# insitro/FastVim

Measured on AMD Instinct MI355X. Metric: images/sec FastVim-T 224px bs=128/GPU fwd+bwd (+all-reduce +AdamW +EMA), whole job, higher is better.
Workload: dtype bf16; 1 GPU; FastVim-T 224x224 bs=128/GPU bf16 training step, synthetic ImageNet tensors (BASELINE configs[1]); global_batch=128, parallelism=dp1, hip_graph=True, optimizer_in_step=True, final_loss_hex=0x1.779ca20000000p+0

## Files before the change

fastvim_amd/_lib.py:

```python
import ctypes
import os
import threading

import torch

_PKG = os.path.dirname(os.path.abspath(__file__))
LIB_PATH = os.path.join(_PKG, "libfastvim_hip.so")

FV_F32, FV_BF16, FV_F16 = 0, 1, 2
_DTYPES = {torch.float32: FV_F32, torch.bfloat16: FV_BF16, torch.float16: FV_F16}

_lib = None

C_ABI_SYMBOLS = (
    "fv_last_error", "fv_version",
    "fv_selective_scan_fwd", "fv_selective_scan_bwd_workspace", "fv_selective_scan_bwd",
    "fv_causal_conv1d_fwd", "fv_causal_conv1d_bwd", "fv_scan_expand_skip_fwd",
    "fv_mixer_conv_pool_fwd", "fv_mixer_scan_fwd", "fv_mixer_xproj_scan_fwd_ok", "fv_mixer_xproj_scan_fwd", "fv_mixer_combine_fwd",
    "fv_mixer_bwd_blocks", "fv_mixer_combine_bwd", "fv_mixer_scan_bwd_chunks", "fv_mixer_scan_bwd_chunks_b",
    "fv_mixer_scan_bwd_ckpt_floats", "fv_mixer_scan_bwd_partials", "fv_mixer_scan_bwd", "fv_mixer_scan_bwd_dir", "fv_mixer_scan_bwd_ckpt", "fv_mixer_scan_bwd_segments", "fv_mixer_scan_bwd_seg_floats", "fv_mixer_scan_bwd_seg_partials", "fv_mixer_scan_bwd_seg_chunks", "fv_mixer_scan_bwd_seg", "fv_mixer_scan_fwd_ckpt", "fv_mixer_scan_ckpt_floats", "fv_mixer_scan_fwd_segments", "fv_mixer_scan_fwd_seg_floats", "fv_mixer_scan_fwd_seg", "fv_rows_segment_sum", "fv_rows_gather", "fv_mixer_conv_pool_bwd", "fv_mixer_conv_pool_bwd2_ok", "fv_mixer_conv_pool_bwd2", "fv_mixer_scan_bwd_xproj_ok", "fv_mixer_scan_bwd_xproj", "fv_chunk_rows_bf16", "fv_reduce_partials", "fv_reduce_partials_multi",
    "fv_add_norm_blocks", "fv_add_norm_fwd", "fv_add_norm_bwd", "fv_gemm_bf16", "fv_gemm_bf16_tn_grouped", "fv_gemm_bf16_tn_grouped_ld", "fv_mixer_xproj_fwd", "fv_mixer_xproj_bwd_slices", "fv_mixer_xproj_bwd", "fv_mixer_xproj_bwd2", "fv_mixer_xproj_bwd3_ok", "fv_mixer_xproj_bwd3", "fv_adamw_flat", "fv_soft_target_ce",
    "fv_patch_unfold", "fv_gemm_bf16_rowbias", "fv_mean_pool_fwd", "fv_mean_pool_bwd", "fv_droppath_table", "fv_scale_cast",
    "fv_column_sum", "fv_gemm_bf16_addnorm", "fv_gemm_bf16_dgrad_addnorm_blocks", "fv_gemm_bf16_dgrad_addnorm_bwd", "fv_gemm_bf16_dgrad_addnorm_bwd2", "fv_gemm_bf16_addnorm2", "fv_mixer_combine_out_proj_addnorm_ok", "fv_mixer_combine_out_proj_addnorm", "fv_gemm_f32",
    "fv_mixer_conv_pool_bwd_dgrad_ok", "fv_mixer_conv_pool_bwd_dgrad_blocks", "fv_mixer_conv_pool_bwd_dgrad", "fv_transpose_bf16_batched", "fv_gemm_bf16_tn_grouped_wide8",
    "fv_grad_sumsq_blocks", "fv_grad_sumsq_partials", "fv_adamw_flat_groups",
    "fv_pack_weight_frags_batched", "fv_mixer_conv_pool_bwd_dgrad_pk", "fv_mixer_combine_out_proj_addnorm_pk",
    "fv_mix_batch", "fv_patch_unfold_mix", "fv_mixup_target", "fv_label_ce",
    "fv_patch_unfold_chan", "fv_chan_embed_table", "fv_chan_embed_scatter",
    "fv_mixer_plan",
    "fv_bn1d_stats", "fv_bn1d_apply", "fv_bn1d_bwd", "fv_sgd_flat", "fv_lars_partials_per_segment", "fv_lars_sumsq_partials", "fv_lars_flat",
    "fv_tap_ln_blocks", "fv_tap_ln_fwd", "fv_tap_ln_bwd", "fv_ln2d_blocks", "fv_ln2d_fwd", "fv_ln2d_bwd",
)


_tls = threading.local()


class _DeviceGuarded:

    def __init__(self, cdll):
        self._cdll = cdll
        self._wrapped = {}

    def __getattr__(self, name):
        w = self._wrapped.get(name)
        if w is None:
            fn = getattr(self._cdll, name)

            def call(*args, _fn=fn):
                dev = getattr(_tls, "dev", None)
                if dev is None or dev == torch.cuda.current_device():
                    return _fn(*args)
                with torch.cuda.device(dev):
                    return _fn(*args)

            w = self._wrapped[name] = call
        return w


def lib():
    global _lib
    if _lib is None:
        if not os.path.exists(LIB_PATH):
            raise RuntimeError(
# ... 44 lines not shown
```

fastvim_amd/csrc/scan_cl.hip:

```cpp
#include <stdlib.h>

#include "common.h"
#include "lane_reduce.h"
#include "scan_step.h"
#include <type_traits>

namespace {

constexpr int N = 16;
constexpr int CPB = 64;

struct ScanClParams {
  const void* xc;
  const void* xdbl;
  const float* Wdt[2];
  const float* dtb[2];
  const float* Alog[2];
  float* yc;
  const float* dyc;
  size_t dyc_dir;
  float* dxc;
  float* dxdbl;
  float* ckpt;
  float* pP;
// ... 1327 lines not shown
  }
}

__global__ __launch_bounds__(256) void scan_seg_combine_kernel(ScanClParams p) {
  const size_t i = (size_t)blockIdx.x * blockDim.x + threadIdx.x;
  const size_t per = (size_t)p.d_in * N, total = (size_t)2 * p.B * per;
  if (i >= total) return;
  const int n = (int)(i % N), d = (int)((i / N) % p.d_in);
  const size_t db = i / per;
  const int dir = (int)(db / p.B);
  const float A = -__expf(p.Alog[dir][(size_t)d * N + n]);
  float* hin = const_cast<float*>(p.hin);
  float H = 0.f;
  for (int k = 0; k < p.seg; ++k) {
    const int s = p.adj ? p.seg - 1 - k : k;
    const size_t sidx = (db * p.seg + s) * p.d_in + d;
    hin[sidx * N + n] = H;
    H = fmaf(__expf(A * p.sumdt[sidx]), H, p.hend[sidx * N + n]);
  }
}

typedef __bf16 sc_bf16x8 __attribute__((ext_vector_type(8)));

template <int RQ, int LCT>
struct ShortFwdLds {
  static constexpr int RQP = (RQ + 3) / 4 * 4, WP = 4 * RQP + 2 * N;
  static constexpr int xc_stride(int d_in) { return d_in * 2 + 16; }
  static constexpr int o_xc = 0;
  static constexpr int o_dbl(int d_in) { return o_xc + 16 * xc_stride(d_in); }
  static constexpr int o_ch(int d_in) { return o_dbl(d_in) + LCT * WP * 4; }
  static constexpr int o_y(int d_in) { return o_ch(d_in) + LCT * SH_CH * 8; }
  static constexpr int o_xp(int d_in) { return o_y(d_in) + LCT * SH_CH * 4; }
  static constexpr int bytes(int d_in, int NT) { return o_xp(d_in) + SH_NWV * NT * 256 * 4; }
};

template <int RQ, int LCT, bool EXACT>
__global__ __launch_bounds__(SH_THREADS) void xproj_scan_fwd_short_kernel(ScanClParams p, const bf16_t* __restrict__ Wx2,
                                                                         bf16_t* __restrict__ xdbl_out, int NT) {
  extern __shared__ __attribute__((aligned(16))) char smc[];
  typedef ShortFwdLds<RQ, LCT> LD;
  constexpr int RQP = LD::RQP, WP = LD::WP;
  const int d_in = p.d_in, W = p.R + 2 * N;
  const int Lc = EXACT ? LCT : p.Lc;
  const int XS = LD::xc_stride(d_in);
  char* s_xc = smc + LD::o_xc;
  float* s_dbl = (float*)(smc + LD::o_dbl(d_in));
  float* s_ch = (float*)(smc + LD::o_ch(d_in));
  float* s_y = (float*)(smc + LD::o_y(d_in));
  float* s_xp = (float*)(smc + LD::o_xp(d_in));
  const int tid = threadIdx.x, lane = tid & 63, wv = tid >> 6;
  const int dir = blockIdx.y, b = blockIdx.x;
  const size_t bd = ((size_t)dir * p.B + b) * Lc;
  struct ChunkPar { float w[RQP]; float bias; float al[4]; };
  auto load_par = [&](int ch0, ChunkPar& c) {
    const int dm = ch0 + wv * 16 + (lane & 15), tg_ = lane >> 4;
    const bool actm = dm < d_in;
    const int ddm = actm ? dm : 0;
    c.bias = p.dtb[dir][ddm];
#pragma unroll
    for (int kg = 0; kg < RQP; ++kg) {
      const int r = 4 * kg + tg_;
      c.w[kg] = (actm && r < p.R) ? p.Wdt[dir][(size_t)ddm * p.R + r] : 0.f;
    }
    const int d = ch0 + wv * 16 + (lane >> 2), dd = d < d_in ? d : 0;
    const float4 a4 = *reinterpret_cast<const float4*>(p.Alog[dir] + (size_t)dd * N + (lane & 3) * 4);
    c.al[0] = a4.x; c.al[1] = a4.y; c.al[2] = a4.z; c.al[3] = a4.w;
  };
  ChunkPar par0, par1;
  load_par(0, par0);
  if (SH_CH < d_in) load_par(SH_CH, par1);
  sc_bf16x8 bw0[7];
  {
    const int r = lane & 15, kc = lane >> 4;
    const bf16_t* Wd = Wx2 + (size_t)dir * W * d_in;
    const int k0 = min(wv, d_in / 32 - 1) * 32 + kc * 8;
#pragma unroll
    for (int nt = 0; nt < 7; ++nt)
      if (nt < NT) bw0[nt] = *reinterpret_cast<const sc_bf16x8*>(Wd + (size_t)min(nt * 16 + r, W - 1) * d_in + k0);
  }
  {
    const bf16_t* xc = (const bf16_t*)p.xc + bd * d_in;
    const int vpr = d_in / 8;
    for (int e = tid; e < 16 * vpr; e += SH_THREADS) {
      const int srow = e / vpr, v = e - srow * vpr;
      uint4 val = make_uint4(0u, 0u, 0u, 0u);
      if (srow < Lc) {
        const int l = dir ? Lc - 1 - srow : srow;
        val = *reinterpret_cast<const uint4*>(xc + (size_t)l * d_in + v * 8);
      }
      *reinterpret_cast<uint4*>(s_xc + srow * XS + v * 16) = val;
    }
    for (int e = tid; e < LCT * WP; e += SH_THREADS) s_dbl[e] = 0.f;
  }
  __syncthreads();
  {
    f32x4_t acc[7];
#pragma unroll
    for (int nt = 0; nt < 7; ++nt) acc[nt] = (f32x4_t){0.f, 0.f, 0.f, 0.f};
    const int r = lane & 15, kc = lane >> 4;
    const bf16_t* Wd = Wx2 + (size_t)dir * W * d_in;
    for (int ks = wv; ks < d_in / 32; ks += SH_NWV) {
      const int k0 = ks * 32 + kc * 8;
      const sc_bf16x8 a = *reinterpret_cast<const sc_bf16x8*>(s_xc + r * XS + k0 * 2);
#pragma unroll
      for (int nt = 0; nt < 7; ++nt) {
        if (nt < NT) {
          const int n = min(nt * 16 + r, W - 1);
          const sc_bf16x8 bw = ks == wv ? bw0[nt] : *reinterpret_cast<const sc_bf16x8*>(Wd + (size_t)n * d_in + k0);
          acc[nt] = __builtin_amdgcn_mfma_f32_16x16x32_bf16(bw, a, acc[nt], 0, 0, 0);
        }
      }
    }
#pragma unroll
    for (int nt = 0; nt < 7; ++nt)
      if (nt < NT) *reinterpret_cast<f32x4_t*>(s_xp + ((size_t)(wv * NT + nt) * 64 + lane) * 4) = acc[nt];
  }
  __syncthreads();
  {
    bf16_t* xo = xdbl_out + bd * W;
    for (int e = tid; e < Lc * W; e += SH_THREADS) {
      const int t = e / W, n = e - t * W;
      const int nt = n >> 4, ln = t + 16 * ((n & 15) >> 2), j = n & 3;
      float v = 0.f;
#pragma unroll
      for (int w = 0; w < SH_NWV; ++w) v += s_xp[((size_t)(w * NT + nt) * 64 + ln) * 4 + j];
      const bf16_t vb = __float2bfloat16(v);
      const int l = dir ? Lc - 1 - t : t;
      xo[(size_t)l * W + n] = vb;
      const int pos = n < p.R ? (n & 3) * RQP + (n >> 2) : 4 * RQP + (n - p.R);
      s_dbl[t * WP + pos] = __bfloat162float(vb);
    }
  }
  __syncthreads();
  const int q = lane & 3, cm = lane & 15, tg = lane >> 4;
  const float* my_bc = s_dbl + 4 * RQP + q * 4;
  auto chunk = [&](int ch0, const ChunkPar& par) {
    {
      const int dm = ch0 + wv * 16 + cm;
      const bool actm = dm < d_in;
      const int ddm = actm ? dm : 0;
      const float bias_m = par.bias;
      f32x4_t D = {0.f, 0.f, 0.f, 0.f};
      const int ta = min(cm, LCT - 1);
#pragma unroll
      for (int kg = 0; kg < RQP; ++kg) {
        const float a = s_dbl[ta * WP + tg * RQP + kg];
        D = __builtin_amdgcn_mfma_f32_16x16x4f32(a, par.w[kg], D, 0, 0, 0);
// ... 29 lines not shown
        asm volatile("" ::: "memory");
        if (EXACT || s < Lc) {
          const float4 Bv = *reinterpret_cast<const float4*>(my_bc + s * WP);
          const float4 Cv = *reinterpret_cast<const float4*>(my_bc + s * WP + N);
          const float2 cv = *reinterpret_cast<const float2*>(my_ch + s * (SH_CH * 2));
          const sf2 Bn[2] = {{Bv.x, Bv.y}, {Bv.z, Bv.w}}, Cn[2] = {{Cv.x, Cv.y}, {Cv.z, Cv.w}};
          sf2 acc2 = {0.f, 0.f};
#pragma unroll
          for (int h = 0; h < 2; ++h) {
            st[h] = sfma2(sexp2_2(A2[h] * cv.x), st[h], Bn[h] * cv.y);
            acc2 = sfma2(Cn[h], st[h], acc2);
          }
          const float acc = quad_sum(acc2.x + acc2.y);
          s_y[s * SH_CH + chl] = acc;
        }
      }
    }
    __builtin_amdgcn_fence(__ATOMIC_RELEASE, "wavefront");
    __builtin_amdgcn_wave_barrier();
    __builtin_amdgcn_fence(__ATOMIC_ACQUIRE, "wavefront");
    {
      const int dm = ch0 + wv * 16 + cm;
#pragma unroll
      for (int r = 0; r < 4; ++r) {
        const int s = 4 * tg + r;
        if (dm < d_in && s < Lc) {
          const int l = dir ? Lc - 1 - s : s;
          p.yc[(bd + l) * d_in + dm] = s_y[s * SH_CH + wv * 16 + cm];
        }
      }
    }
    __builtin_amdgcn_wave_barrier();
  };
  chunk(0, par0);
  if (SH_CH < d_in) chunk(SH_CH, par1);
  for (int ch0 = 2 * SH_CH; ch0 < d_in; ch0 += SH_CH) {
    ChunkPar pc;
    load_par(ch0, pc);
    chunk(ch0, pc);
  }
}

int rq_of(int R) { return (R + 3) / 4; }

}

extern "C" int fv_mixer_scan_fwd(const void* xc, const void* x_dbl, const float* dt_w, const float* dt_bias,
                                 const float* A_log, const float* dt_w_b, const float* dt_bias_b,
                                 const float* A_log_b, float* yc, int batch, int Lc, int d_inner, int dt_rank,
                                 int d_state, int dtype, fv_stream_t stream) {
  return fv_mixer_scan_fwd_ckpt(xc, x_dbl, dt_w, dt_bias, A_log, dt_w_b, dt_bias_b, A_log_b, yc, nullptr, batch, Lc, d_inner,
                                dt_rank, d_state, dtype, stream);
}

extern "C" int fv_mixer_scan_fwd_segments(int batch, int Lc, int d_inner, int dt_rank) {
  static const int force = fv_tune("FASTVIM_SCAN_FWD_SEG", 0);
  const int nchunk = (Lc + 15) / 16;
  if (Lc <= 16 || dt_rank > 48) return 1;
  if (force > 0) {
    const int f = force < nchunk ? force : nchunk, cps = (nchunk + f - 1) / f;
    return (nchunk + cps - 1) / cps;
  }
  const long wgs = (long)fv_cdiv(d_inner, CPB) * batch * 2;
  if (wgs >= 512 || nchunk < 16) return 1;
  long s = (1024 + wgs - 1) / wgs;
  if (s > nchunk / 8) s = nchunk / 8;
  if (s < 1) s = 1;
  const long cps = (nchunk + s - 1) / s;
  return (int)((nchunk + cps - 1) / cps);
}
extern "C" size_t fv_mixer_scan_fwd_seg_floats(int batch, int Lc, int d_inner, int d_state, int dt_rank) {
  const int S = fv_mixer_scan_fwd_segments(batch, Lc, d_inner, dt_rank);
// ... 89 lines not shown
           Lc, d_inner, dt_rank);
  FV_CHECK(xc && x_proj_w2 && dt_w && dt_bias && A_log && dt_w_b && dt_bias_b && A_log_b && x_dbl && yc,
           "mixer_xproj_scan_fwd: null pointer");
  FV_CHECK(((uintptr_t)xc & 15) == 0 && ((uintptr_t)x_proj_w2 & 15) == 0 && d_inner % 8 == 0,
           "mixer_xproj_scan_fwd: operands must be 16-byte aligned");
  ScanClParams p{};
  p.xc = xc; p.yc = yc;
  p.Wdt[0] = dt_w; p.Wdt[1] = dt_w_b; p.dtb[0] = dt_bias; p.dtb[1] = dt_bias_b;
  p.Alog[0] = A_log; p.Alog[1] = A_log_b;
  p.B = batch; p.Lc = Lc; p.d_in = d_inner; p.R = dt_rank;
  const int RQ = rq_of(dt_rank), NT = fv_cdiv(dt_rank + 2 * N, 16);
  dim3 grid(batch, 2), block(SH_THREADS);
  hipStream_t st = (hipStream_t)stream;
#define FV_XS(RQQ, LCC, EXX)                                                                 \
  do {                                                                                       \
    const size_t smem = (size_t)ShortFwdLds<RQQ, LCC>::bytes(d_inner, NT);                   \
    static FvOncePerDevice done;                                                                   \
    if (done.first()) {                                                                             \
      (void)hipFuncSetAttribute((const void*)xproj_scan_fwd_short_kernel<RQQ, LCC, EXX>,     \
                                hipFuncAttributeMaxDynamicSharedMemorySize, 160 * 1024);     \
      (void)0;                                                                                \
    }                                                                                        \
    hipLaunchKernelGGL((xproj_scan_fwd_short_kernel<RQQ, LCC, EXX>), grid, block, smem, st, p, \
                       (const bf16_t*)x_proj_w2, (bf16_t*)x_dbl, NT);                        \
  } while (0)
#define FV_XSL(RQQ)                                                                          \
  do {                                                                                       \
    if (Lc == 14) FV_XS(RQQ, 14, true); else if (Lc < 14) FV_XS(RQQ, 14, false);             \
    else if (Lc == 16) FV_XS(RQQ, 16, true); else FV_XS(RQQ, 16, false);                     \
  } while (0)
  if (RQ <= 3) FV_XSL(3); else if (RQ <= 6) FV_XSL(6); else FV_XSL(12);
#undef FV_XSL
#undef FV_XS
  FV_LAUNCH_CHECK();
  return FV_OK;
}

static bool bwd_short(int Lc, int dt_rank) {
  static const int off = (fv_tune("FASTVIM_SCAN_SHORT", 1) == 0);
  return Lc <= 16 && dt_rank <= 48 && !off;
}
static bool bwd_chunked(int Lc, int dt_rank) {
  static const int off = (fv_tune("FASTVIM_SCAN_CHUNKED", 1) == 0);
  return Lc > 16 && dt_rank <= 48 && !off;
}
extern "C" size_t fv_mixer_scan_ckpt_floats(int batch, int Lc, int d_inner, int d_state, int dt_rank) {
  return bwd_chunked(Lc, dt_rank) ? (size_t)2 * batch * ((Lc + 15) / 16) * d_inner * d_state : 0;
}

static int ck_waves(int batch, int d_inner) {
  static const int force = fv_tune("FASTVIM_SCAN_CK_WAVES", 0);
  if (force == 4 || force == 12) return force;
  return (long)fv_cdiv(d_inner, 192) * batch * 2 >= 256 ? 12 : 4;
}
extern "C" int fv_mixer_scan_bwd_chunks_b(int batch, int d_inner, int Lc, int dt_rank) {
  return fv_cdiv(d_inner, bwd_short(Lc, dt_rank) ? SH_CH : bwd_chunked(Lc, dt_rank) ? 16 * ck_waves(batch, d_inner) : CPB);
}
extern "C" int fv_mixer_scan_bwd_chunks(int d_inner, int Lc, int dt_rank) {
  return fv_mixer_scan_bwd_chunks_b(1 << 20, d_inner, Lc, dt_rank);
}

static int scan_bwd_nbb(int batch, int Lc, int dt_rank) {
  static const int force = fv_tune("FASTVIM_SCAN_NBB", 0);
  if (force > 0 && batch % force == 0) return force;
  if (!bwd_short(Lc, dt_rank)) return 1;
  const long chunks = fv_cdiv(32 * dt_rank, SH_CH);
// ... 242 lines not shown
```

fastvim_amd/mamba_simple_faster.py:

```python
import ctypes
import math

import torch
import torch.nn as nn
import torch.nn.functional as F

from . import _lib as L
from . import mixer_ops as M
from .gemm import gemm_any_bnn, gemm_any_btn, gemm_any_nn, gemm_any_nt, gemm_any_tn, gemm_nn, gemm_nt, gemm_tn


def _shadow(w, cdt):
    sh = getattr(w, "_fv_shadow", None)
    if sh is not None and sh.dtype == cdt:
        if w._version != w._fv_shadow_version:
            with torch.no_grad():
                sh.copy_(w)
            w._fv_shadow_version = w._version
        return sh
    return w.to(cdt)


def _shadow_t(w, cdt):
    wt = getattr(w, "_fv_shadow_t", None)
    if wt is not None and wt.dtype == cdt:
        if w._version != w._fv_shadow_t_version:
            with torch.no_grad():
                wt.copy_(_shadow(w, cdt).t())
            w._fv_shadow_t_version = w._version
        return wt
    return _shadow(w, cdt).t().contiguous()


class _PackedWeights:
    enabled = True


def use_packed_weights(on):
    was = _PackedWeights.enabled
    _PackedWeights.enabled = bool(on)
    return was

# ... 234 lines not shown
            dres_out = dres_out.reshape(Mrows, d).contiguous() if dres_out is not None else None
            dx = torch.empty(Mrows, d, device=dev, dtype=cdt)
            dres_in = torch.empty(Mrows, d, device=dev, dtype=torch.float32)
            lib = L.lib()
            nb = lib.fv_add_norm_blocks(L.i32(Mrows))
            pw = torch.empty(nb, d, device=dev, dtype=torch.float32)
            rc = lib.fv_add_norm_bwd(
                L.ptr(dy), L.i32(L.dtype_code(dy.dtype)), L.ptr(dres_out),
                L.i32(L.dtype_code(dres_out.dtype) if dres_out is not None else 0), L.ptr(r), L.i32(L.FV_F32),
                L.ptr(w32), L.ptr(None), L.ptr(rstd), L.ptr(row_scale), L.i32(ctx.rows_per_scale), L.ptr(dx),
                L.i32(L.dtype_code(cdt)), L.ptr(dres_in), L.i32(L.FV_F32), L.ptr(pw), L.ptr(None), L.i32(Mrows), L.i32(d),
                L.i32(1), L.stream_of(r))
            L.check(rc, "add_norm_bwd")
            gd = _direct_grad(ctx.w_param)
            if gd is not None:
                M.reduce_partials(pw, nb, out=gd.view(-1), accumulate=True)
                dw = None
            else:
                dw = M.reduce_partials(pw, nb).to(ctx.w_param.dtype)
            g2 = g.view(Mrows, d_in)
            dg = linear_dgrad(dx, _shadow(W_out, cdt)).view(B, Ltok, d_in)
            dW_out = _SideStream.run(lambda: linear_wgrad(dx, g2, W_out), dx, g)
        return dg, dW_out, dres_in.view(B, Ltok, d), dw, None, None, None


class _Ctx:

    def save_for_backward(self, *tensors):
        self.saved_tensors = tensors


COMBINE_IN_OUT_PROJ = True
CONV_IN_DGRAD = True
XPROJ_TWO_ADDENDS = True


def resolve_combine(pack):
    if pack is not None:
        M.combine_fwd(pack["xz"], pack["skip"], pack["yc"], pack["ln_w"], pack["ln_b"], pack["eps"], pack["rows"],
                      pack["cols"], pack["transposed"], out=pack["out"])


def _out_proj_add_norm_fwd(g, W_out, residual, norm_w, eps, row_scale, cdt, W_in=None, pack=None):
    B, Ltok, d_in = g.shape
    d = W_out.shape[0]
    Mrows = B * Ltok
    g2 = g.view(Mrows, d_in)
    res2 = residual.reshape(Mrows, d).contiguous()
    w32 = norm_w.float().contiguous()
    y = torch.empty(Mrows, d, device=g.device, dtype=cdt)
    res_out = torch.empty(Mrows, d, device=g.device, dtype=torch.float32)
    rstd = torch.empty(Mrows, device=g.device, dtype=torch.float32)
    rows_per_scale = 1
    if row_scale is not None:
        row_scale = row_scale.float().contiguous()
        rows_per_scale = Mrows // row_scale.numel()
    xz = None
    if W_in is not None and W_in.shape[0] % 128 == 0:
        xz = torch.empty(Mrows, W_in.shape[0], device=g.device, dtype=cdt)
    W_out_c = _shadow(W_out, cdt)
    W_in_c = _shadow(W_in, cdt) if xz is not None else None
    lib = L.lib()
    if pack is not None:
        if xz is None and W_out_c.stride(1) == 1 and W_out_c.stride(0) % 8 == 0 and W_out_c.data_ptr() % 16 == 0:
            y, res_out, rstd = M.combine_out_proj_addnorm(pack["xz"], pack["skip"], pack["yc"], pack["ln_w"], pack["ln_b"],
                                                          pack["eps"], pack["rows"], pack["cols"], pack["transposed"],
# ... 129 lines not shown
        return torch.float32 if dt == torch.float16 else dt
    return torch.float32 if t.dtype == torch.float16 else t.dtype


def half_io(t):
    if torch.is_autocast_enabled():
        return torch.get_autocast_dtype('cuda') == torch.float16
    return t.dtype == torch.float16


def mixer_apply(fn, hidden, *args):
    if any(torch.is_tensor(a) and a.dtype == torch.float16 for a in args):
        args = tuple(a.float() if torch.is_tensor(a) and a.dtype == torch.float16 else a for a in args)
    out = fn.apply(hidden, *args)
    return out.to(torch.float16) if hidden.dtype == torch.float16 else out


class FastVimMixerFn(torch.autograd.Function):

    @staticmethod
    def forward(ctx, hidden, W_in, b_in, cw, cb, cw_b, cb_b, Wx, Wx_b, Wdt, bdt, Wdt_b, bdt_b, A_log, A_b_log,
                D, D_b, ln_w, ln_b, W_out, b_out, rows, cols, transposed, pool_max, scaling, ln_eps, cdt, fv, tpp=1,
                valid=None):
        L.require_gpu(hidden)
        B, Ltok, d = hidden.shape
        if Ltok != rows * cols * tpp:
            raise RuntimeError(f"Mamba: sequence length {Ltok} != token grid {rows}x{cols}x{tpp}")
        d_in = W_in.shape[0] // 2
        with torch.autocast("cuda", enabled=False):
            h_c = hidden.to(cdt).contiguous()
            W_in_c = _shadow(W_in, cdt)
            W_out_c = _shadow(W_out, cdt) if W_out is not None else None
            xz = getattr(ctx, "precomputed_xz", None)
            if xz is None:
                xz = linear_fwd(h_c.view(B * Ltok, d), W_in_c, b_in)
            xz = xz.view(B, Ltok, 2 * d_in)
            cw2, cwb2 = cw.reshape(d_in, -1), cw_b.reshape(d_in, -1)
            amax = None
            if fv is not None and "Wx2" in fv:
                Wx2 = fv["Wx2"]
                if fv["Wx2_shadow"].dtype == cdt:
                    _shadow(Wx, cdt), _shadow(Wx_b, cdt)
                    Wx2_c = fv["Wx2_shadow"]
                else:
                    Wx2_c = Wx2.to(cdt)
            else:
                Wx2 = torch.stack([Wx, Wx_b])
                Wx2_c = Wx2.to(cdt)
            if pool_max:
                xc, skip, amax = M.conv_pool_fwd(xz, cw2, cb, cwb2, cb_b, rows, cols, transposed, pool_max, scaling, tpp,
                                                 D=D, D_b=D_b)
            else:
                xc, skip = M.conv_pool_fwd(xz, cw2, cb, cwb2, cb_b, rows, cols, transposed, pool_max, scaling, tpp,
                                           D=D, D_b=D_b)
            if valid is not None and valid < rows * tpp:
                xc[:, :, valid:].zero_()
            fused = M.xproj_scan_fwd(xc, Wx2_c, Wdt, bdt, A_log, Wdt_b, bdt_b, A_b_log)
            if fused is not None:
                x_dbl, yc = fused
            else:
                x_dbl = M.xproj_fwd(xc, Wx2_c)
                nig = getattr(ctx, "needs_input_grad", None)
                yc, ctx.scan_ckpt = M.scan_fwd(xc, x_dbl, Wdt, bdt, A_log, Wdt_b, bdt_b, A_b_log,
                                               want_ckpt=nig is None or any(nig))
            if (getattr(ctx, "defer_combine", False) and W_out is None and not pool_max and valid is None
                    and M.combine_out_proj_addnorm_ok(xz, rows, cols, tpp, d)):
                g, mean, rstd = M.combine_buffers(xz, ln_w)
                ctx.pending_combine = dict(xz=xz, skip=skip, yc=yc, ln_w=ln_w, ln_b=ln_b, eps=ln_eps, rows=rows, cols=cols,
                                           transposed=transposed, out=(g, mean, rstd))
            else:
                g, mean, rstd = M.combine_fwd(xz, skip, yc, ln_w, ln_b, ln_eps, rows, cols, transposed, tpp=tpp)
            out = g if W_out is None else linear_fwd(g.view(B * Ltok, d_in), W_out_c, b_out).view(B, Ltok, d)
        ctx.save_for_backward(h_c, W_in, cw, cb, cw_b, cb_b, Wx2, Wdt, bdt, Wdt_b, bdt_b, A_log, A_b_log, D, D_b,
                              ln_w, ln_b, W_out, xz, xc, x_dbl, g, skip, yc, mean, rstd, amax)
        ctx.geo = (rows, cols, transposed, pool_max, scaling, tpp)
        ctx.has_bias = (b_in is not None, b_out is not None)
        ctx.cdt = cdt
        ctx.in_dtype = hidden.dtype
        ctx.fv = fv
        return out

    @staticmethod
    def backward(ctx, dout):
        (h_c, W_in, cw, cb, cw_b, cb_b, Wx2, Wdt, bdt, Wdt_b, bdt_b, A_log, A_b_log, D, D_b, ln_w, ln_b, W_out,
         xz, xc, x_dbl, g, skip, yc, mean, rstd, amax) = ctx.saved_tensors
        rows, cols, transposed, pool_max, scaling, tpp = ctx.geo
        cdt = ctx.cdt
        B, Ltok, d = h_c.shape
        d_in = W_in.shape[0] // 2
        fv = ctx.fv or {}
# ... 214 lines not shown
```

fastvim_amd/mixer_ops.py:

```python
import ctypes

import torch

from . import _lib as L

f32 = ctypes.c_float


def _geo(rows, cols, transposed):
    return (1, rows) if transposed else (cols, 1)


def conv_pool_fwd(xz, conv_w, conv_b, conv_w_b, conv_b_b, rows, cols, transposed, pool_max, scaling, tpp=1,
                  D=None, D_b=None):
    B, Ltok, two_d = xz.shape
    d_in = two_d // 2
    s_i, s_j = _geo(rows, cols, transposed)
    xc = torch.empty(2, B, rows * tpp, d_in, device=xz.device, dtype=xz.dtype)
    skip = torch.empty(B, Ltok, d_in, device=xz.device, dtype=xz.dtype) if D is not None else None
    amax = torch.empty_like(xc) if pool_max else None
    rc = L.lib().fv_mixer_conv_pool_fwd(
        L.ptr(xz), L.ptr(conv_w), L.ptr(conv_b), L.ptr(conv_w_b), L.ptr(conv_b_b), L.ptr(D), L.ptr(D_b), L.ptr(xc),
        L.ptr(skip), L.ptr(amax), L.i32(B), L.i32(rows), L.i32(cols), L.i32(s_i), L.i32(s_j), L.i32(tpp), L.i32(d_in),
        L.i32(conv_w.shape[-1]), L.i32(pool_max), f32(scaling), L.i32(L.dtype_code(xz.dtype)), L.stream_of(xz))
# ... 9 lines not shown
    N = A_log.shape[1]
    lib = L.lib()
    yc = torch.empty(2, B, Lc, d_in, device=xc.device, dtype=torch.float32)
    ckpt = None
    if want_ckpt:
        nck = lib.fv_mixer_scan_ckpt_floats(L.i32(B), L.i32(Lc), L.i32(d_in), L.i32(N), L.i32(R))
        ckpt = torch.empty(nck, device=xc.device, dtype=torch.float32) if nck else None
    nws = lib.fv_mixer_scan_fwd_seg_floats(L.i32(B), L.i32(Lc), L.i32(d_in), L.i32(N), L.i32(R))
    ws = torch.empty(nws, device=xc.device, dtype=torch.float32) if nws else None
    rc = lib.fv_mixer_scan_fwd_seg(
        L.ptr(xc), L.ptr(x_dbl), L.ptr(dt_w), L.ptr(dt_b), L.ptr(A_log), L.ptr(dt_w_b), L.ptr(dt_b_b),
        L.ptr(A_log_b), L.ptr(yc), L.ptr(ckpt), L.ptr(ws), L.i32(B), L.i32(Lc), L.i32(d_in), L.i32(R), L.i32(N),
        L.i32(L.dtype_code(xc.dtype)), L.stream_of(xc))
    L.check(rc, "mixer_scan_fwd")
    return (yc, ckpt) if want_ckpt else yc


def xproj_scan_fwd(xc, Wx2_c, dt_w, dt_b, A_log, dt_w_b, dt_b_b, A_log_b):
    _, B, Lc, d_in = xc.shape
    R, N = dt_w.shape[1], A_log.shape[1]
    W = Wx2_c.shape[1]
    lib = L.lib()
    if (xc.dtype != torch.bfloat16 or Wx2_c.dtype != torch.bfloat16 or N != 16 or W != R + 2 * N
            or not xc.is_contiguous() or not Wx2_c.is_contiguous() or xc.data_ptr() % 16 or Wx2_c.data_ptr() % 16
            or not lib.fv_mixer_xproj_scan_fwd_ok(L.i32(Lc), L.i32(d_in), L.i32(R), L.i32(L.dtype_code(xc.dtype)))):
        return None
    x_dbl = torch.empty(2, B * Lc, W, device=xc.device, dtype=xc.dtype)
    yc = torch.empty(2, B, Lc, d_in, device=xc.device, dtype=torch.float32)
    rc = lib.fv_mixer_xproj_scan_fwd(
        L.ptr(xc), L.ptr(Wx2_c), L.ptr(dt_w), L.ptr(dt_b), L.ptr(A_log), L.ptr(dt_w_b), L.ptr(dt_b_b), L.ptr(A_log_b),
        L.ptr(x_dbl), L.ptr(yc), L.i32(B), L.i32(Lc), L.i32(d_in), L.i32(R), L.i32(N), L.i32(L.dtype_code(xc.dtype)),
        L.stream_of(xc))
    L.check(rc, "mixer_xproj_scan_fwd")
    return x_dbl, yc


def combine_buffers(xz, ln_w):
    B, Ltok, two_d = xz.shape
    g = torch.empty(B, Ltok, two_d // 2, device=xz.device, dtype=xz.dtype)
    if ln_w is not None:
        return g, torch.empty(B * Ltok, device=xz.device, dtype=torch.float32), torch.empty(B * Ltok, device=xz.device, dtype=torch.float32)
    return g, None, None


def combine_fwd(xz, skip, yc, ln_w, ln_b, eps, rows, cols, transposed, tpp=1, out=None):
    B, Ltok, two_d = xz.shape
    d_in = two_d // 2
    s_i, s_j = _geo(rows, cols, transposed)
    g, mean, rstd = out if out is not None else combine_buffers(xz, ln_w)
    rc = L.lib().fv_mixer_combine_fwd(
        L.ptr(xz), L.ptr(skip), L.ptr(yc), L.ptr(ln_w), L.ptr(ln_b), f32(eps), L.ptr(g), L.ptr(mean), L.ptr(rstd),
        L.i32(B), L.i32(rows), L.i32(cols), L.i32(s_i), L.i32(s_j), L.i32(tpp), L.i32(d_in),
        L.i32(L.dtype_code(xz.dtype)), L.stream_of(xz))
    L.check(rc, "mixer_combine_fwd")
    return g, mean, rstd


class _Deferred:
    enabled = False
    max_jobs = 144
    side = False
    jobs = []
    stream = None
    pending = []

    @classmethod
# ... 414 lines not shown
```

include/fastvim_hip.h:

```cpp
#ifndef FASTVIM_HIP_H
#define FASTVIM_HIP_H

#include <stddef.h>
#include <stdint.h>

#ifdef __cplusplus
extern "C" {
#endif

typedef void* fv_stream_t;

enum { FV_F32 = 0, FV_BF16 = 1, FV_F16 = 2 };
enum { FV_OK = 0, FV_ERR_INVALID = -1, FV_ERR_HIP = -2, FV_ERR_UNSUPPORTED = -3 };

const char* fv_last_error(void);
#define FV_ABI_VERSION 3
int fv_version(void);

int fv_selective_scan_fwd(const void* u, const void* delta, const float* A, const void* B,
                          const void* C, const float* D, const void* z, const float* delta_bias,
                          void* out, float* last_state, int batch, int dim, int seqlen, int dstate,
                          int n_groups, int B_variable, int C_variable, int delta_softplus,
                          int dtype, fv_stream_t stream);

// ... 13 lines not shown
                         float* partials, int batch, int dim, int seqlen, int width, int silu, int dtype,
                         fv_stream_t stream);

int fv_scan_expand_skip_fwd(const void* yc, const void* u_full, const float* D, void* out, int batch, int dim,
                            int seqlen, int seqlen_compressed, int dtype, fv_stream_t stream);

int fv_mixer_conv_pool_fwd(const void* xz, const float* conv_w, const float* conv_b,
                           const float* conv_w_b, const float* conv_b_b, const float* D, const float* D_b,
                           void* xc, void* skip, void* amax, int batch, int rows, int cols, int tok_stride_row,
                           int tok_stride_col, int tokens_per_patch, int d_inner, int d_conv, int pool_max,
                           float scaling_factor, int dtype, fv_stream_t stream);

int fv_mixer_scan_fwd(const void* xc, const void* x_dbl, const float* dt_w, const float* dt_bias,
                      const float* A_log, const float* dt_w_b, const float* dt_bias_b,
                      const float* A_log_b, float* yc, int batch, int Lc, int d_inner, int dt_rank,
                      int d_state, int dtype, fv_stream_t stream);
size_t fv_mixer_scan_ckpt_floats(int batch, int Lc, int d_inner, int d_state, int dt_rank);
int fv_mixer_scan_fwd_ckpt(const void* xc, const void* x_dbl, const float* dt_w, const float* dt_bias,
                           const float* A_log, const float* dt_w_b, const float* dt_bias_b,
                           const float* A_log_b, float* yc, float* ckpt, int batch, int Lc, int d_inner, int dt_rank,
                           int d_state, int dtype, fv_stream_t stream);
int fv_mixer_scan_fwd_segments(int batch, int Lc, int d_inner, int dt_rank);
size_t fv_mixer_scan_fwd_seg_floats(int batch, int Lc, int d_inner, int d_state, int dt_rank);
int fv_mixer_scan_fwd_seg(const void* xc, const void* x_dbl, const float* dt_w, const float* dt_bias,
                          const float* A_log, const float* dt_w_b, const float* dt_bias_b, const float* A_log_b,
                          float* yc, float* ckpt, float* seg_ws, int batch, int Lc, int d_inner, int dt_rank,
                          int d_state, int dtype, fv_stream_t stream);

int fv_mixer_xproj_scan_fwd_ok(int Lc, int d_inner, int dt_rank, int dtype);
int fv_mixer_xproj_scan_fwd(const void* xc, const void* x_proj_w2, const float* dt_w, const float* dt_bias,
                            const float* A_log, const float* dt_w_b, const float* dt_bias_b, const float* A_log_b,
                            void* x_dbl, float* yc, int batch, int Lc, int d_inner, int dt_rank, int d_state,
                            int dtype, fv_stream_t stream);

int fv_mixer_combine_fwd(const void* xz, const void* skip, const float* yc, const float* ln_w,
                         const float* ln_b, float ln_eps, void* g, float* mean, float* rstd, int batch,
                         int rows, int cols, int tok_stride_row, int tok_stride_col, int tokens_per_patch,
                         int d_inner, int dtype, fv_stream_t stream);

int fv_mixer_bwd_blocks(int batch, int rows, int d_inner, int tokens_per_patch, int which);

int fv_mixer_plan(int family, int batch, int rows, int cols, int tokens_per_patch, int d_inner, int pool_max, int dtype,
                  int* plan);

int fv_mixer_combine_bwd(const void* dg, const void* xz, const void* skip, const float* yc,
                         const float* ln_w, const float* ln_b, const float* mean, const float* rstd,
                         void* dxz, void* d_o, float* dyc, float* partials, int batch, int rows, int cols, int tok_stride_row,
                         int tok_stride_col, int tokens_per_patch, int d_inner, int dtype, fv_stream_t stream);

int fv_mixer_scan_bwd_chunks(int d_inner, int Lc, int dt_rank);
int fv_mixer_scan_bwd_chunks_b(int batch, int d_inner, int Lc, int dt_rank);
int fv_mixer_scan_bwd_partials(int batch, int Lc, int dt_rank);
size_t fv_mixer_scan_bwd_ckpt_floats(int batch, int Lc, int d_inner, int d_state, int dt_rank);
int fv_mixer_scan_bwd(const void* xc, const void* x_dbl, const float* dt_w, const float* dt_bias,
                      const float* A_log, const float* dt_w_b, const float* dt_bias_b, const float* A_log_b,
                      const float* dyc, float* dxc, float* dx_dbl, float* ckpt, float* partials, int batch,
                      int Lc, int d_inner, int dt_rank, int d_state, int dtype, fv_stream_t stream);
int fv_mixer_scan_bwd_dir(const void* xc, const void* x_dbl, const float* dt_w, const float* dt_bias,
                          const float* A_log, const float* dt_w_b, const float* dt_bias_b, const float* A_log_b,
                          const float* dyc, int dyc_per_direction, float* dxc, float* dx_dbl, float* ckpt,
                          float* partials, int batch, int Lc, int d_inner, int dt_rank, int d_state, int dtype,
                          fv_stream_t stream);
int fv_mixer_scan_bwd_ckpt(const void* xc, const void* x_dbl, const float* dt_w, const float* dt_bias,
                           const float* A_log, const float* dt_w_b, const float* dt_bias_b, const float* A_log_b,
                           const float* dyc, int dyc_per_direction, float* dxc, float* dx_dbl, float* ckpt,
                           int ckpt_given, float* partials, int batch, int Lc, int d_inner, int dt_rank, int d_state,
// ... 231 lines not shown
```

Measured before the change: 25980 images/sec.

## Co-schedule z-half input projection GEMM with short xproj+scan kernel

The in_proj GEMM now computes only the x half up front. The z half (columns d_in..2*d_in) runs inside the same launch as the fused x_proj+selective-scan forward, in extra workgroups beyond the scan blocks, so the small GEMM fills CUs the scan leaves idle and one launch is saved. The scan body is templated with a compile-time NT, an LDS layout where the xproj scratch aliases the chunk tables, and an optional late parameter load, to cut LDS and register pressure. This adds complexity and shape restrictions (d_model 192, d_inner 384, tpp 1). It also risks slowing the scan through shared occupancy or LDS limits.

```diff
diff --git a/fastvim_amd/_lib.py b/fastvim_amd/_lib.py
--- a/fastvim_amd/_lib.py
+++ b/fastvim_amd/_lib.py
@@ -30,6 +30,7 @@
     "fv_mixer_plan",
     "fv_bn1d_stats", "fv_bn1d_apply", "fv_bn1d_bwd", "fv_sgd_flat", "fv_lars_partials_per_segment", "fv_lars_sumsq_partials", "fv_lars_flat",
     "fv_tap_ln_blocks", "fv_tap_ln_fwd", "fv_tap_ln_bwd", "fv_ln2d_blocks", "fv_ln2d_fwd", "fv_ln2d_bwd",
+    "fv_mixer_xproj_scan_fwd_zproj_ok", "fv_mixer_xproj_scan_fwd_zproj_lds_bytes", "fv_mixer_xproj_scan_fwd_zproj",
 )
 
 
diff --git a/fastvim_amd/csrc/scan_cl.hip b/fastvim_amd/csrc/scan_cl.hip
--- a/fastvim_amd/csrc/scan_cl.hip
+++ b/fastvim_amd/csrc/scan_cl.hip
@@ -1383,14 +1383,20 @@
   static constexpr int o_y(int d_in) { return o_ch(d_in) + LCT * SH_CH * 8; }
   static constexpr int o_xp(int d_in) { return o_y(d_in) + LCT * SH_CH * 4; }
   static constexpr int bytes(int d_in, int NT) { return o_xp(d_in) + SH_NWV * NT * 256 * 4; }
+  static constexpr int bytes_alias(int d_in, int NT) {
+    const int xp = SH_NWV * NT * 256 * 4, tab = LCT * SH_CH * 12;
+    return o_ch(d_in) + (xp > tab ? xp : tab);
+  }
 };
 
-template <int RQ, int LCT, bool EXACT>
-__global__ __launch_bounds__(SH_THREADS) void xproj_scan_fwd_short_kernel(ScanClParams p, const bf16_t* __restrict__ Wx2,
-                                                                         bf16_t* __restrict__ xdbl_out, int NT) {
+template <int RQ, int LCT, bool EXACT, int NTC = 0, bool ALIAS = false, bool PAR1_LATE = false>
+__device__ __forceinline__ void xproj_scan_fwd_short_body(const ScanClParams& p, const bf16_t* __restrict__ Wx2,
+                                                          bf16_t* __restrict__ xdbl_out, int NT_rt, int dir, int b) {
   extern __shared__ __attribute__((aligned(16))) char smc[];
   typedef ShortFwdLds<RQ, LCT> LD;
   constexpr int RQP = LD::RQP, WP = LD::WP;
+  constexpr int NTM = NTC > 0 ? NTC : 7;
+  const int NT = NTC > 0 ? NTC : NT_rt;
   const int d_in = p.d_in, W = p.R + 2 * N;
   const int Lc = EXACT ? LCT : p.Lc;
   const int XS = LD::xc_stride(d_in);
@@ -1398,9 +1404,8 @@
   float* s_dbl = (float*)(smc + LD::o_dbl(d_in));
   float* s_ch = (float*)(smc + LD::o_ch(d_in));
   float* s_y = (float*)(smc + LD::o_y(d_in));
-  float* s_xp = (float*)(smc + LD::o_xp(d_in));
+  float* s_xp = (float*)(smc + (ALIAS ? LD::o_ch(d_in) : LD::o_xp(d_in)));
   const int tid = threadIdx.x, lane = tid & 63, wv = tid >> 6;
-  const int dir = blockIdx.y, b = blockIdx.x;
   const size_t bd = ((size_t)dir * p.B + b) * Lc;
   struct ChunkPar { float w[RQP]; float bias; float al[4]; };
   auto load_par = [&](int ch0, ChunkPar& c) {
@@ -1419,14 +1424,14 @@
   };
   ChunkPar par0, par1;
   load_par(0, par0);
-  if (SH_CH < d_in) load_par(SH_CH, par1);
-  sc_bf16x8 bw0[7];
+  if (!PAR1_LATE && SH_CH < d_in) load_par(SH_CH, par1);
+  sc_bf16x8 bw0[NTM];
   {
     const int r = lane & 15, kc = lane >> 4;
     const bf16_t* Wd = Wx2 + (size_t)dir * W * d_in;
     const int k0 = min(wv, d_in / 32 - 1) * 32 + kc * 8;
 #pragma unroll
-    for (int nt = 0; nt < 7; ++nt)
+    for (int nt = 0; nt < NTM; ++nt)
       if (nt < NT) bw0[nt] = *reinterpret_cast<const sc_bf16x8*>(Wd + (size_t)min(nt * 16 + r, W - 1) * d_in + k0);
   }
   {
@@ -1445,16 +1450,16 @@
   }
   __syncthreads();
   {
-    f32x4_t acc[7];
-#pragma unroll
-    for (int nt = 0; nt < 7; ++nt) acc[nt] = (f32x4_t){0.f, 0.f, 0.f, 0.f};
+    f32x4_t acc[NTM];
+#pragma unroll
+    for (int nt = 0; nt < NTM; ++nt) acc[nt] = (f32x4_t){0.f, 0.f, 0.f, 0.f};
     const int r = lane & 15, kc = lane >> 4;
     const bf16_t* Wd = Wx2 + (size_t)dir * W * d_in;
     for (int ks = wv; ks < d_in / 32; ks += SH_NWV) {
       const int k0 = ks * 32 + kc * 8;
       const sc_bf16x8 a = *reinterpret_cast<const sc_bf16x8*>(s_xc + r * XS + k0 * 2);
 #pragma unroll
-      for (int nt = 0; nt < 7; ++nt) {
+      for (int nt = 0; nt < NTM; ++nt) {
         if (nt < NT) {
           const int n = min(nt * 16 + r, W - 1);
           const sc_bf16x8 bw = ks == wv ? bw0[nt] : *reinterpret_cast<const sc_bf16x8*>(Wd + (size_t)n * d_in + k0);
@@ -1463,7 +1468,7 @@
       }
     }
 #pragma unroll
-    for (int nt = 0; nt < 7; ++nt)
+    for (int nt = 0; nt < NTM; ++nt)
       if (nt < NT) *reinterpret_cast<f32x4_t*>(s_xp + ((size_t)(wv * NT + nt) * 64 + lane) * 4) = acc[nt];
   }
   __syncthreads();
@@ -1559,12 +1564,112 @@
     }
     __builtin_amdgcn_wave_barrier();
   };
+  if (PAR1_LATE && SH_CH < d_in) load_par(SH_CH, par1);
   chunk(0, par0);
   if (SH_CH < d_in) chunk(SH_CH, par1);
   for (int ch0 = 2 * SH_CH; ch0 < d_in; ch0 += SH_CH) {
     ChunkPar pc;
     load_par(ch0, pc);
     chunk(ch0, pc);
+  }
+}
+
+template <int RQ, int LCT, bool EXACT>
+__global__ __launch_bounds__(SH_THREADS) void xproj_scan_fwd_short_kernel(ScanClParams p, const bf16_t* __restrict__ Wx2,
+                                                                         bf16_t* __restrict__ xdbl_out, int NT) {
+  xproj_scan_fwd_short_body<RQ, LCT, EXACT>(p, Wx2, xdbl_out, NT, blockIdx.y, blockIdx.x);
+}
+
+
+struct ZProjParams {
+  const bf16_t* y;
+  const bf16_t* W;
+  bf16_t* xz;
+  const float* bias;
+  int M, tiles, nwg;
+};
+constexpr int ZP_K = 192, ZP_N = 384, ZP_LDC = 768, ZP_BM = 64;
+constexpr int ZP_AS = ZP_K * 2 + 16;
+constexpr int ZP_TILE = ZP_BM * ZP_AS;
+constexpr int ZP_VPT = ZP_BM * (ZP_K / 8) / SH_THREADS;
+static_assert(ZP_N == 2 * 16 * SH_NWV, "two column halves of one 16-column slice per wave");
+static_assert(ZP_VPT * SH_THREADS == ZP_BM * (ZP_K / 8), "whole vectors per thread");
+
+__device__ __forceinline__ void zproj_role(const ZProjParams& z, int g) {
+  extern __shared__ __attribute__((aligned(16))) char smz[];
+  const int tid = threadIdx.x, lane = tid & 63, wv = tid >> 6;
+  const int r = lane & 15, kc = lane >> 4;
+  const int ts = z.nwg >> 1;
+  int t = g >> 1;
+  if (t >= z.tiles) return;
+  const int n0 = (g & 1) * (ZP_N / 2) + wv * 16;
+  sc_bf16x8 fb[ZP_K / 32];
+  {
+    const bf16_t* Wl = z.W + (size_t)(n0 + r) * ZP_K + kc * 8;
+#pragma unroll
+    for (int ks = 0; ks < ZP_K / 32; ++ks) fb[ks] = *reinterpret_cast<const sc_bf16x8*>(Wl + ks * 32);
+  }
+  const int n = n0 + kc * 4;
+  float4 bj = make_float4(0.f, 0.f, 0.f, 0.f);
+  if (z.bias) bj = *reinterpret_cast<const float4*>(z.bias + n);
+  uint4 st[ZP_VPT];
+  auto fetch = [&](int tt) {
+#pragma unroll
+    for (int i = 0; i < ZP_VPT; ++i) {
+      const int e = tid + i * SH_THREADS, row = e / (ZP_K / 8), v = e - row * (ZP_K / 8);
+      st[i] = make_uint4(0u, 0u, 0u, 0u);
+      if (tt * ZP_BM + row < z.M) st[i] = *reinterpret_cast<const uint4*>(z.y + (size_t)(tt * ZP_BM + row) * ZP_K + v * 8);
+    }
+  };
+  auto put = [&](int buf) {
+#pragma unroll
+    for (int i = 0; i < ZP_VPT; ++i) {
+      const int e = tid + i * SH_THREADS, row = e / (ZP_K / 8), v = e - row * (ZP_K / 8);
+      *reinterpret_cast<uint4*>(smz + buf * ZP_TILE + row * ZP_AS + v * 16) = st[i];
+    }
+  };
+  fetch(t);
+  put(0);
+  __syncthreads();
+  for (int buf = 0; t < z.tiles; t += ts, buf ^= 1) {
+    const bool more = t + ts < z.tiles;
+    if (more) fetch(t + ts);
+    f32x4_t acc[4];
+#pragma unroll
+    for (int b = 0; b < 4; ++b) acc[b] = (f32x4_t){0.f, 0.f, 0.f, 0.f};
+    const char* sa = smz + buf * ZP_TILE + r * ZP_AS + kc * 16;
+#pragma unroll
+    for (int ks = 0; ks < ZP_K / 32; ++ks) {
+      sc_bf16x8 fa[4];
+#pragma unroll
+      for (int b = 0; b < 4; ++b) fa[b] = *reinterpret_cast<const sc_bf16x8*>(sa + b * 16 * ZP_AS + ks * 64);
+#pragma unroll
+      for (int b = 0; b < 4; ++b) acc[b] = __builtin_amdgcn_mfma_f32_16x16x32_bf16(fb[ks], fa[b], acc[b], 0, 0, 0);
+    }
+#pragma unroll
+    for (int b = 0; b < 4; ++b) {
+      const int m = t * ZP_BM + b * 16 + r;
+      f32x4_t v = acc[b];
+      if (z.bias) { v[0] += bj.x; v[1] += bj.y; v[2] += bj.z; v[3] += bj.w; }
+      if (m < z.M) {
+        const uint2 pk = {pack_bf16x2(v[0], v[1]), pack_bf16x2(v[2], v[3])};
+        *reinterpret_cast<uint2*>(z.xz + (size_t)m * ZP_LDC + n) = pk;
+      }
+    }
+    if (more) put(buf ^ 1);
+    __syncthreads();
+  }
+}
+
+template <int LCT, bool EXACT>
+__global__ __launch_bounds__(SH_THREADS, 6) void xproj_scan_fwd_zproj_kernel(ScanClParams p, const bf16_t* __restrict__ Wx2,
+                                                                            bf16_t* __restrict__ xdbl_out, ZProjParams z) {
+  const int id = blockIdx.x, nscan = 2 * p.B;
+  if (id < nscan) {
+    const int dir = id >= p.B ? 1 : 0;
+    xproj_scan_fwd_short_body<3, LCT, EXACT, 3, true>(p, Wx2, xdbl_out, 3, dir, id - dir * p.B);
+  } else {
+    zproj_role(z, id - nscan);
   }
 }
 
@@ -1720,6 +1825,61 @@
   if (RQ <= 3) FV_XSL(3); else if (RQ <= 6) FV_XSL(6); else FV_XSL(12);
 #undef FV_XSL
 #undef FV_XS
+  FV_LAUNCH_CHECK();
+  return FV_OK;
+}
+
+extern "C" int fv_mixer_xproj_scan_fwd_zproj_ok(int Lc, int d_model, int d_inner, int dt_rank, int tpp, int dtype) {
+  return Lc >= 1 && Lc <= 16 && d_model == ZP_K && d_inner == ZP_N && dt_rank >= 1 && dt_rank <= 12 && tpp == 1 &&
+         dtype == FV_BF16 && fv_cdiv(dt_rank + 2 * N, 16) == 3;
+}
+extern "C" int fv_mixer_xproj_scan_fwd_zproj_lds_bytes(int Lc, int d_inner) {
+  const int scan = Lc <= 14 ? ShortFwdLds<3, 14>::bytes_alias(d_inner, 3) : ShortFwdLds<3, 16>::bytes_alias(d_inner, 3);
+  const int gemm = 2 * ZP_TILE;
+  return scan > gemm ? scan : gemm;
+}
+
+extern "C" int fv_mixer_xproj_scan_fwd_zproj(const void* xc, const void* x_proj_w2, const float* dt_w, const float* dt_bias,
+                                             const float* A_log, const float* dt_w_b, const float* dt_bias_b,
+                                             const float* A_log_b, void* x_dbl, float* yc, const void* y, const void* w_in,
+                                             const float* b_in, void* xz, int batch, int Lc, int d_model, int d_inner,
+                                             int dt_rank, int d_state, int tokens, int gemm_wgs, int dtype,
+                                             fv_stream_t stream) {
+  FV_CHECK(d_state == N, "mixer_xproj_scan_fwd_zproj: only d_state == 16 is built (got %d)", d_state);
+  FV_CHECK(batch > 0 && fv_mixer_xproj_scan_fwd_zproj_ok(Lc, d_model, d_inner, dt_rank, 1, dtype),
+           "mixer_xproj_scan_fwd_zproj: needs bf16, d_model 192, d_inner 384, Lc <= 16, dt_rank <= 12 (got Lc %d, d_model %d, "
+           "d_inner %d, dt_rank %d)", Lc, d_model, d_inner, dt_rank);
+  FV_CHECK(xc && x_proj_w2 && dt_w && dt_bias && A_log && dt_w_b && dt_bias_b && A_log_b && x_dbl && yc,
+           "mixer_xproj_scan_fwd_zproj: null pointer");
+  FV_CHECK(((uintptr_t)xc & 15) == 0 && ((uintptr_t)x_proj_w2 & 15) == 0, "mixer_xproj_scan_fwd_zproj: operands must be 16-byte aligned");
+  ZProjParams z{};
+  if (gemm_wgs != 0) {
+    FV_CHECK(y && w_in && xz && tokens > 0, "mixer_xproj_scan_fwd_zproj: null GEMM operand");
+    FV_CHECK(((uintptr_t)y & 15) == 0 && ((uintptr_t)w_in & 15) == 0 && ((uintptr_t)xz & 15) == 0 && ((uintptr_t)b_in & 15) == 0,
+             "mixer_xproj_scan_fwd_zproj: GEMM operands must be 16-byte aligned");
+    z.y = (const bf16_t*)y;
+    z.W = (const bf16_t*)w_in + (size_t)ZP_N * ZP_K;
+    z.xz = (bf16_t*)xz + ZP_N;
+    z.bias = b_in ? b_in + ZP_N : nullptr;
+    z.M = tokens;
+    z.tiles = fv_cdiv(tokens, ZP_BM);
+    const int per_half = gemm_wgs < 0 ? (fv_cu_count() / 2 > 0 ? fv_cu_count() / 2 : 1) : gemm_wgs;
+    z.nwg = 2 * (per_half > z.tiles ? z.tiles : per_half);
+  }
+  ScanClParams p{};
+  p.xc = xc; p.yc = yc;
+  p.Wdt[0] = dt_w; p.Wdt[1] = dt_w_b; p.dtb[0] = dt_bias; p.dtb[1] = dt_bias_b;
+  p.Alog[0] = A_log; p.Alog[1] = A_log_b;
+  p.B = batch; p.Lc = Lc; p.d_in = d_inner; p.R = dt_rank;
+  const dim3 grid(2 * batch + z.nwg), block(SH_THREADS);
+  const size_t smem = (size_t)fv_mixer_xproj_scan_fwd_zproj_lds_bytes(Lc, d_inner);
+  hipStream_t st = (hipStream_t)stream;
+#define FV_XZ(LCC, EXX)                                                                                  \
+  hipLaunchKernelGGL((xproj_scan_fwd_zproj_kernel<LCC, EXX>), grid, block, smem, st, p, (const bf16_t*)x_proj_w2, \
+                     (bf16_t*)x_dbl, z)
+  if (Lc == 14) FV_XZ(14, true); else if (Lc < 14) FV_XZ(14, false);
+  else if (Lc == 16) FV_XZ(16, true); else FV_XZ(16, false);
+#undef FV_XZ
   FV_LAUNCH_CHECK();
   return FV_OK;
 }
diff --git a/fastvim_amd/mamba_simple_faster.py b/fastvim_amd/mamba_simple_faster.py
--- a/fastvim_amd/mamba_simple_faster.py
+++ b/fastvim_amd/mamba_simple_faster.py
@@ -8,6 +8,7 @@
 from . import _lib as L
 from . import mixer_ops as M
 from .gemm import gemm_any_bnn, gemm_any_btn, gemm_any_nn, gemm_any_nt, gemm_any_tn, gemm_nn, gemm_nt, gemm_tn
+from .gemm import _call as gemm_call
 
 
 def _shadow(w, cdt):
@@ -308,6 +309,7 @@
 
 COMBINE_IN_OUT_PROJ = True
 CONV_IN_DGRAD = True
+SCAN_ZPROJ = True
 XPROJ_TWO_ADDENDS = True
 
 
@@ -503,8 +505,18 @@
             W_in_c = _shadow(W_in, cdt)
             W_out_c = _shadow(W_out, cdt) if W_out is not None else None
             xz = getattr(ctx, "precomputed_xz", None)
+            zproj = None
             if xz is None:
-                xz = linear_fwd(h_c.view(B * Ltok, d), W_in_c, b_in)
+                h2 = h_c.view(B * Ltok, d)
+                b32 = None if b_in is None else b_in.float()
+                if (SCAN_ZPROJ and cdt == torch.bfloat16 and _mfma_ok(h2, W_in_c) and W_in_c.is_contiguous()
+                        and L.lib().fv_mixer_xproj_scan_fwd_zproj_ok(L.i32(rows * tpp), L.i32(d), L.i32(d_in), L.i32(Wdt.shape[1]),
+                                                                     L.i32(tpp), L.i32(L.FV_BF16))):
+                    xz = torch.empty(B * Ltok, 2 * d_in, device=h_c.device, dtype=cdt)
+                    gemm_call(h2, W_in_c, xz, b32, B * Ltok, d_in, d, d, d, 2 * d_in, 0, 0, 1)
+                    zproj = (h2, b32)
+                else:
+                    xz = linear_fwd(h2, W_in_c, b_in)
             xz = xz.view(B, Ltok, 2 * d_in)
             cw2, cwb2 = cw.reshape(d_in, -1), cw_b.reshape(d_in, -1)
             amax = None
@@ -526,7 +538,15 @@
                                            D=D, D_b=D_b)
             if valid is not None and valid < rows * tpp:
                 xc[:, :, valid:].zero_()
-            fused = M.xproj_scan_fwd(xc, Wx2_c, Wdt, bdt, A_log, Wdt_b, bdt_b, A_b_log)
+            fused = None
+            if zproj is not None:
+                fused = M.xproj_scan_fwd_zproj(xc, Wx2_c, Wdt, bdt, A_log, Wdt_b, bdt_b, A_b_log, zproj[0], W_in_c, zproj[1],
+                                               xz.view(B * Ltok, 2 * d_in), tpp=tpp, gemm_wgs=0 if SCAN_ZPROJ == 2 else -1)
+                if fused is None or SCAN_ZPROJ == 2:
+                    gemm_call(zproj[0], W_in_c[d_in:], xz.view(B * Ltok, 2 * d_in)[:, d_in:],
+                              None if zproj[1] is None else zproj[1][d_in:], B * Ltok, d_in, d, d, d, 2 * d_in, 0, 0, 1)
+            if fused is None:
+                fused = M.xproj_scan_fwd(xc, Wx2_c, Wdt, bdt, A_log, Wdt_b, bdt_b, A_b_log)
             if fused is not None:
                 x_dbl, yc = fused
             else:
diff --git a/fastvim_amd/mixer_ops.py b/fastvim_amd/mixer_ops.py
--- a/fastvim_amd/mixer_ops.py
+++ b/fastvim_amd/mixer_ops.py
@@ -65,6 +65,30 @@
         L.ptr(x_dbl), L.ptr(yc), L.i32(B), L.i32(Lc), L.i32(d_in), L.i32(R), L.i32(N), L.i32(L.dtype_code(xc.dtype)),
         L.stream_of(xc))
     L.check(rc, "mixer_xproj_scan_fwd")
+    return x_dbl, yc
+
+
+def xproj_scan_fwd_zproj(xc, Wx2_c, dt_w, dt_b, A_log, dt_w_b, dt_b_b, A_log_b, y2, W_in_c, b_in, xz, tpp=1, gemm_wgs=-1):
+    _, B, Lc, d_in = xc.shape
+    R, N = dt_w.shape[1], A_log.shape[1]
+    W = Wx2_c.shape[1]
+    tokens, d = y2.shape
+    lib = L.lib()
+    ts = (xc, Wx2_c, y2, W_in_c, xz)
+    if (any(t.dtype != torch.bfloat16 or not t.is_contiguous() or t.data_ptr() % 16 for t in ts) or N != 16 or W != R + 2 * N
+            or tuple(W_in_c.shape) != (2 * d_in, d) or tuple(xz.shape) != (tokens, 2 * d_in)
+            or (b_in is not None and (b_in.dtype != torch.float32 or not b_in.is_contiguous() or b_in.data_ptr() % 16
+                                      or b_in.numel() != 2 * d_in))
+            or not lib.fv_mixer_xproj_scan_fwd_zproj_ok(L.i32(Lc), L.i32(d), L.i32(d_in), L.i32(R), L.i32(tpp),
+                                                        L.i32(L.dtype_code(xc.dtype)))):
+        return None
+    x_dbl = torch.empty(2, B * Lc, W, device=xc.device, dtype=xc.dtype)
+    yc = torch.empty(2, B, Lc, d_in, device=xc.device, dtype=torch.float32)
+    rc = lib.fv_mixer_xproj_scan_fwd_zproj(
+        L.ptr(xc), L.ptr(Wx2_c), L.ptr(dt_w), L.ptr(dt_b), L.ptr(A_log), L.ptr(dt_w_b), L.ptr(dt_b_b), L.ptr(A_log_b),
+        L.ptr(x_dbl), L.ptr(yc), L.ptr(y2), L.ptr(W_in_c), L.ptr(b_in), L.ptr(xz), L.i32(B), L.i32(Lc), L.i32(d), L.i32(d_in),
+        L.i32(R), L.i32(N), L.i32(tokens), L.i32(gemm_wgs), L.i32(L.dtype_code(xc.dtype)), L.stream_of(xc))
+    L.check(rc, "mixer_xproj_scan_fwd_zproj")
     return x_dbl, yc
 
 
diff --git a/include/fastvim_hip.h b/include/fastvim_hip.h
--- a/include/fastvim_hip.h
+++ b/include/fastvim_hip.h
@@ -69,6 +69,14 @@
                             const float* A_log, const float* dt_w_b, const float* dt_bias_b, const float* A_log_b,
                             void* x_dbl, float* yc, int batch, int Lc, int d_inner, int dt_rank, int d_state,
                             int dtype, fv_stream_t stream);
+
+int fv_mixer_xproj_scan_fwd_zproj_ok(int Lc, int d_model, int d_inner, int dt_rank, int tokens_per_patch, int dtype);
+int fv_mixer_xproj_scan_fwd_zproj_lds_bytes(int Lc, int d_inner);
+int fv_mixer_xproj_scan_fwd_zproj(const void* xc, const void* x_proj_w2, const float* dt_w, const float* dt_bias,
+                                  const float* A_log, const float* dt_w_b, const float* dt_bias_b, const float* A_log_b,
+                                  void* x_dbl, float* yc, const void* y, const void* w_in, const float* b_in, void* xz,
+                                  int batch, int Lc, int d_model, int d_inner, int dt_rank, int d_state, int tokens,
+                                  int gemm_wgs, int dtype, fv_stream_t stream);
 
 int fv_mixer_combine_fwd(const void* xz, const void* skip, const float* yc, const float* ln_w,
                          const float* ln_b, float ln_eps, void* g, float* mean, float* rstd, int batch,
```

After: 25720 images/sec. 1.0% lower.
